# WGLab/NanoRepeat

Hardware: NVIDIA B200
Metric: GCUPS (higher is better)
Workload: dtype u16x2 (2*score + mark + 64 per half, two reads per word); s32 (score*65536 - span) for reads > 384 bases

## Files before the change

nanorepeat_b200/csrc/nr_launch_pair2.cu:

```cuda
#define NR_DEFINE_PAIR_ROUND2_KERNEL
#include "nr_launch.h"
#include <mutex>
namespace nrl {
cudaError_t launch_pair_round2(int blocks, int threads, size_t smem, cudaStream_t st, const nr::pr::Pair2* pairs,
                               const nr::pr::Deal& deal, const nr::Task* tasks, const nr::RestArgs& ra, const uint32_t* pool,
                               const nr::ScoreW& k, int* counter, int stride, int4* out, uint32_t* state) {
    static std::mutex mu;
    static bool done = false;
    {
        std::lock_guard<std::mutex> lk(mu);
        cudaError_t e = prepare(nr::pr::pair_round2_kernel, done);
        if (e != cudaSuccess) return e;
    }
    nr::pr::pair_round2_kernel<<<blocks, threads, smem, st>>>(pairs, deal, tasks, ra, pool, k, counter, stride, out, state);
    return cudaGetLastError();
}
}
```

nanorepeat_b200/csrc/nr_launch_pair3.cu:

```cuda
#define NR_DEFINE_PAIR_LADDER_KERNEL
#include "nr_launch.h"
#include <mutex>
namespace nrl {
cudaError_t launch_pair_ladder(int blocks, int threads, size_t smem, cudaStream_t st, const nr::pr::Pair3* pairs,
                               const nr::pr::Deal& deal, const nr::LadderTask* tasks, const nr::RestArgs& ra,
                               const uint32_t* qpool, const uint32_t* pool, const nr::LadderRegion* regs, const nr::ScoreW& k,
                               int* counter, int stride, uint2* prung, int4* out, int4* sel, int* redo_count, int32_t* redo,
                               const uint32_t* qstate) {
    static std::mutex mu;
    static bool done = false;
    {
        std::lock_guard<std::mutex> lk(mu);
        cudaError_t e = prepare(nr::pr::pair_ladder_kernel, done);
        if (e != cudaSuccess) return e;
    }
    nr::pr::pair_ladder_kernel<<<blocks, threads, smem, st>>>(pairs, deal, tasks, ra, qpool, pool, regs, k, counter, stride, prung,
                                                             out, sel, redo_count, redo, qstate);
    return cudaGetLastError();
}
}
```

nanorepeat_b200/csrc/nr_pair_kernels.cuh:

```cuda
#pragma once
#include "nr_kernels.cuh"

namespace nr {
namespace pr {

typedef unsigned u32;
constexpr int kBias = 64;
__host__ __device__ constexpr u32 pk2(int hi, int lo) { return ((u32)(hi & 0xffff) << 16) | (u32)(lo & 0xffff); }
__host__ __device__ constexpr u32 pk(int v) { return pk2(v, v); }
__host__ __device__ constexpr u32 sub2(int v) { return 0u - (((u32)v << 16) | (u32)v); }

constexpr int kMatch = 4, kMismatch = 8, kAmbiguous = 2, kOpen1 = 12, kExt1 = 4, kOpen2 = 50, kExt2 = 2, kRefund1 = 8, kRefund2 = 48;
constexpr u32 kFloorFwd = pk(kBias + 1);
constexpr u32 kFloorBwd = pk(kBias);
constexpr u32 kOnes = 0x00010001u;

__device__ __forceinline__ u32 pmadd(u32 a, u32 mul, u32 b) {
    u32 d;
    asm("mad.lo.u32 %0, %1, %2, %3;" : "=r"(d) : "r"(a), "r"(mul), "r"(b));
    return d;
}

template <u32 FLOOR>
__device__ __forceinline__ void cell(u32 hd, u32 s, u32 one, u32& h, u32& e1, u32& e2, u32& f1, u32& f2) {
    const u32 d = __viaddmax_u16x2(hd, s, FLOOR);
    const u32 t = __vimax3_u16x2(d, e1, e2);
    h = __vimax3_u16x2(t, f1, f2);
    e1 = __viaddmax_u16x2(h, pk(-kOpen1), pmadd(e1, one, sub2(kExt1)));
    e2 = __viaddmax_u16x2(h, pk(-kOpen2), pmadd(e2, one, sub2(kExt2)));
    f1 = __viaddmax_u16x2(h, pk(-kOpen1), pmadd(f1, one, sub2(kExt1)));
    f2 = __viaddmax_u16x2(h, pk(-kOpen2), pmadd(f2, one, sub2(kExt2)));
}

struct Pair2 {
    int32_t a, b;
    int32_t mark_col;
    int32_t state_off;
};

struct Pair3 {
    int32_t a, b;
    int32_t rung_off;
    int32_t state_off;
    int32_t R;
    int32_t pad[3];
};

__host__ __device__ constexpr int state_words(int R) { return 3 * R + 1; }

template <int R>
__device__ __forceinline__ void build_profile(uint4* prof, const uint32_t* __restrict__ qa, int q_a,
                                              const uint32_t* __restrict__ qb, int q_b, int row0, int lane, bool reverse) {
    constexpr int CH = StripeCfg<R>::CH;
    u32* p = reinterpret_cast<u32*>(prof);
    const uint32_t amb_a = q_a > 0 ? read_ambiguity_plane(qa, q_a) : 0u, amb_b = q_b > 0 ? read_ambiguity_plane(qb, q_b) : 0u;
#pragma unroll
    for (int r = 0; r < 4 * CH; ++r) {
        const int i = row0 + r;
        int ca = 4, cb = 4;
        if (r < R && i < q_a) {
            const int qi = reverse ? q_a - 1 - i : i;
            ca = (qa[qi >> 4] >> (30 - 2 * (qi & 15))) & 3;
            if (amb_a && read_base_ambiguous(qa, amb_a, qi)) ca = 5;
        }
        if (r < R && i < q_b) {
            const int qi = reverse ? q_b - 1 - i : i;
            cb = (qb[qi >> 4] >> (30 - 2 * (qi & 15))) & 3;
            if (amb_b && read_base_ambiguous(qb, amb_b, qi)) cb = 5;
        }
#pragma unroll
        for (int c = 0; c < 4; ++c)
            p[((c * CH + (r >> 2)) * 32 + lane) * 4 + (r & 3)] =
                pk2(ca == 5 ? -kAmbiguous : ca == c ? kMatch : -kMismatch, cb == 5 ? -kAmbiguous : cb == c ? kMatch : -kMismatch);
    }
}

constexpr int kP2 = 0, kPB = 1, kPF = 2;

template <int R, int MODE, bool MULTI = false>
struct Sweep {
    static constexpr u32 FLOOR = MODE == kPB ? kFloorBwd : kFloorFwd;
    static constexpr bool kMarks = MODE != kPB;
    bool top, bot;
    const ulonglong2* bnd_in;
    ulonglong2* bnd_out;
    int tag_in, tag_out;
    int* spin;
    int4 bcur;
    ulonglong2 bnxt;
    const ulonglong2* tok_in;
    ulonglong2* tok_out;
    const u32* bstage;
    int b_stride, brow0;
    const int* bdone;
    int bdone_need;
    bool late_pending;
    u32* bsm_w;
    const uint4* prof;
    const uint32_t* twords;
    int t_len, lane;
    int mark_col;
    int q_a, q_b;
    const u32* bsm;
    uint2* rung_out;
    int jnext, m, kcnt, zone_start;
    int col0;
    const u32* resume;
    u32* save;
    int save_col;
    u32 H[R], E1[R], E2[R];
    u32 hup_prev, h_out, f1_out, f2_out;
    u32 best;
    u32 bestc, raw_hi, raw_lo;
    int st_hi, st_lo;
    u32 nz, bz;
    uint32_t twl, w0, w1;
    int wi, wmax, wsh;
    const char* prof_lane;
    u32 tokP, tokJ;

    __device__ __forceinline__ uint32_t tword(int i) const { return __ldg(&twords[min(max(i, 0), wmax)]); }

    __device__ __forceinline__ void init() {
        if (MODE == kPF && resume) {
#pragma unroll
            for (int r = 0; r < R; ++r) {
                H[r] = __ldcg(&resume[r * 32 + lane]);
                E1[r] = __ldcg(&resume[(R + r) * 32 + lane]);
                E2[r] = __ldcg(&resume[(2 * R + r) * 32 + lane]);
            }
            hup_prev = lane ? __ldcg(&resume[(R - 1) * 32 + lane - 1]) : FLOOR;
            best = __ldcg(&resume[3 * R * 32 + lane]);
        } else {
#pragma unroll
            for (int r = 0; r < R; ++r) { H[r] = FLOOR; E1[r] = FLOOR + sub2(kOpen1); E2[r] = FLOOR + sub2(kOpen2); }
            hup_prev = FLOOR;
            best = 0;
        }
        h_out = FLOOR; f1_out = FLOOR; f2_out = FLOOR;
        bestc = FLOOR | kOnes; raw_hi = 0; raw_lo = 0; st_hi = 0; st_lo = 0;
        nz = lane != 0; bz = lane != 0 ? 0u : FLOOR;
        wmax = (t_len + 15) >> 4;
        wi = (col0 - lane) >> 4;
        wsh = 2 * ((col0 - lane) & 15);
        w0 = tword(wi); w1 = tword(wi + 1);
        twl = 0;
        prof_lane = reinterpret_cast<const char*>(prof + lane);
        tokP = 0; tokJ = 0;
        if (MULTI) {
            bcur = make_int4(0, 0, 0, 0); bnxt = make_ulonglong2(0ull, 0ull);
            if (top) bnxt = load_bnd(&bnd_in[lane < t_len ? lane : t_len - 1]);
            late_pending = MODE == kPF;
        }
    }

    __device__ __forceinline__ void refill() {
        twl = __funnelshift_l(w1, w0, wsh);
        w0 = w1;
        ++wi;
        w1 = tword(wi + 1);
    }

    __device__ __forceinline__ unsigned next_base(unsigned four) {
        unsigned lo, hi;
        asm("{\n\t.reg .u64 p;\n\tmul.wide.u32 p, %2, %3;\n\tmov.b64 {%0, %1}, p;\n\t}" : "=r"(lo), "=r"(hi) : "r"(twl), "r"(four));
        twl = lo;
        return hi;
    }

    template <bool JUNC, bool KEEP_E = false>
    __device__ __forceinline__ u32 cells(const uint4* pp, u32 hd, u32 cm, u32& f1, u32& f2, u32 one, u32& jhi, bool keep = false) {
        constexpr int CH = StripeCfg<R>::CH;
        u32 jprev = 0;
#pragma unroll
        for (int c = 0; c < CH; ++c) {
            const uint4 sv = pp[c * 32];
            const u32 s4[4] = {sv.x, sv.y, sv.z, sv.w};
#pragma unroll
            for (int u = 0; u < 4; ++u) {
                const int r = 4 * c + u;
                if (r < R) {
                    const u32 hleft = H[r];
                    const u32 e1pre = E1[r], e2pre = E2[r];
                    u32 h;
                    cell<FLOOR>(hd, s4[u], one, h, E1[r], E2[r], f1, f2);
                    if (KEEP_E) { E1[r] = keep ? e1pre : E1[r]; E2[r] = keep ? e2pre : E2[r]; }
                    if (JUNC) {
                        const u32 bx = bsm[(0 * R + r) * 32 + lane], by = bsm[(1 * R + r) * 32 + lane], bz = bsm[(2 * R + r) * 32 + lane];
                        const u32 t = __vimax3_u16x2(pmadd(h, one, bx), pmadd(e1pre, one, by), pmadd(e2pre, one, bz));
                        if (r & 1) jhi = __vimax3_u16x2(jhi, jprev, t);
                        else if (r == R - 1) jhi = __vmaxu2(jhi, t);
                        jprev = t;
                    }
                    hd = hleft;
                    H[r] = h;
                    if (r & 1) cm = __vimax3_u16x2(cm, h, H[r - 1]);
                    else if (r == R - 1) cm = __vmaxu2(cm, h);
                }
            }
        }
        return cm;
    }

    __device__ __forceinline__ void mark_started_inside() {
#pragma unroll
        for (int r = 0; r < R; ++r) {
            H[r] = __viaddmax_u16x2(H[r], pk(-1), FLOOR);
            E1[r] = __viaddmax_u16x2(E1[r], pk(-1), __vminu2(E1[r], FLOOR));
            E2[r] = __viaddmax_u16x2(E2[r], pk(-1), __vminu2(E2[r], FLOOR));
        }
        hup_prev = __viaddmax_u16x2(hup_prev, pk(-1), FLOOR);
    }

    __device__ __forceinline__ void late_load() {
        wait_cols(bdone, bdone_need, lane, spin);
#pragma unroll
        for (int r = 0; r < R; ++r) {
            const int idx0 = brow0 + lane * R + r;
            const int ia = q_a - 2 - idx0, ib = q_b - 2 - idx0;
#pragma unroll
            for (int c = 0; c < 3; ++c) {
                const u32 da = c == 0 ? (idx0 < q_a ? (u32)kBias : 0u) : 0u, db = c == 0 ? (idx0 < q_b ? (u32)kBias : 0u) : 0u;
                const u32 a = ia >= 0 ? __ldcg(&bstage[c * b_stride + ia]) >> 16 : da;
                const u32 b = ib >= 0 ? __ldcg(&bstage[c * b_stride + ib]) & 0xffffu : db;
                bsm_w[(c * R + r) * 32 + lane] = (a << 16) | b;
            }
        }
        __syncwarp();
        late_pending = false;
    }

    __device__ __forceinline__ void store_stage(u32* stage, int stride, int row0) {
#pragma unroll
        for (int r = 0; r < R; ++r) {
            const int i = row0 + lane * R + r;
            __stcg(&stage[0 * stride + i], H[r]);
            __stcg(&stage[1 * stride + i], E1[r] + pk(kRefund1));
            __stcg(&stage[2 * stride + i], E2[r] + pk(kRefund2));
        }
    }

    __device__ __forceinline__ void store_junction_vectors(u32* stage, u32* bvec_fwd) {
        __syncwarp();
#pragma unroll
        for (int r = 0; r < R; ++r) {
            stage[(0 * R + r) * 32 + lane] = H[r];
            stage[(1 * R + r) * 32 + lane] = E1[r] + pk(kRefund1);
            stage[(2 * R + r) * 32 + lane] = E2[r] + pk(kRefund2);
        }
        __syncwarp();
#pragma unroll
        for (int r = 0; r < R; ++r) {
            const int idx0 = lane * R + r;
            const int ia = q_a - 2 - idx0, ib = q_b - 2 - idx0;
#pragma unroll
            for (int c = 0; c < 3; ++c) {
                const u32 da = c == 0 ? (idx0 < q_a ? (u32)kBias : 0u) : 0u, db = c == 0 ? (idx0 < q_b ? (u32)kBias : 0u) : 0u;
                const u32 a = ia >= 0 ? stage[(c * R + ia % R) * 32 + ia / R] >> 16 : da;
                const u32 b = ib >= 0 ? stage[(c * R + ib % R) * 32 + ib / R] & 0xffffu : db;
                bvec_fwd[(c * R + r) * 32 + lane] = (a << 16) | b;
            }
        }
    }

    template <bool FAST, bool TRACK, bool SPECIAL = false>
    __device__ __forceinline__ void step(int st, u32 one, unsigned four) {
        const bool zone = MODE == kPF && (FAST ? SPECIAL : st >= zone_start);
        constexpr int CH = StripeCfg<R>::CH;
        u32 hup = __shfl_up_sync(kFull, h_out, 1);
        u32 f1 = __shfl_up_sync(kFull, f1_out, 1);
        u32 f2 = __shfl_up_sync(kFull, f2_out, 1);
        u32 tP = 0, tJ = 0;
        if (zone) {
            tP = __shfl_up_sync(kFull, tokP, 1);
            tJ = __shfl_up_sync(kFull, tokJ, 1);
        }
        if (MULTI && top) {
            if ((st & 31) == 0) {
                ulonglong2 raw = bnxt;
                const int cj = st + lane;
                for (int tries = 0; !__all_sync(kFull, bnd_valid(raw, tag_in) || cj >= t_len); ++tries) {
                    if (tries > kSpinLimit) { *spin = 1; break; }
                    if (tries > 3) __nanosleep(32);
                    raw = load_bnd(&bnd_in[cj < t_len ? cj : t_len - 1]);
                }
                bcur = unpack_bnd(raw);
                const int nj = st + 32 + lane;
                bnxt = load_bnd(&bnd_in[nj < t_len ? nj : t_len - 1]);
            }
            const u32 bh = __shfl_sync(kFull, (u32)bcur.x, st & 31);
            const u32 bf1 = __shfl_sync(kFull, (u32)bcur.y, st & 31);
            const u32 bf2 = __shfl_sync(kFull, (u32)bcur.z, st & 31);
            if (lane == 0) { hup = bh; f1 = bf1; f2 = bf2; }
        } else {
            hup = pmadd(hup, nz, bz);
            f1 = pmadd(f1, nz, bz);
            f2 = pmadd(f2, nz, bz);
        }
        const unsigned tb = next_base(four);
        const int rel = st - lane;
        const int jj = rel + col0;
        const bool anyj = zone && __any_sync(kFull, jj + 1 == jnext && jj < t_len);
        if (FAST || (rel >= 0 && jj < t_len)) {
            const uint4* pp = reinterpret_cast<const uint4*>(prof_lane + tb * (unsigned)(CH * 512));
            const u32 hd = hup_prev;
            hup_prev = hup;
            constexpr bool kChecks = !FAST || SPECIAL;
            const bool last_col = !FAST && MODE == kPB && jj == t_len - 1;
            u32 cm, jhi = 0;
            const u32 cm0 = (MODE == kP2 && TRACK) ? 0u : best;
            if (zone && anyj) cm = cells<true>(pp, hd, cm0, f1, f2, one, jhi);
            else if (MODE == kPB && !FAST) cm = cells<false, true>(pp, hd, cm0, f1, f2, one, jhi, last_col);
            else cm = cells<false>(pp, hd, cm0, f1, f2, one, jhi);
            h_out = H[R - 1]; f1_out = f1; f2_out = f2;
            if (MODE == kP2 && TRACK) {
                const u32 nb = __vmaxu2(bestc, cm | kOnes);
                const u32 x = nb ^ bestc;
                bestc = nb;
                if (x > 0xffffu) { st_hi = st; raw_hi = cm; }
                if (x & 0xffffu) { st_lo = st; raw_lo = cm; }
                if (kChecks && save && jj == save_col) {
#pragma unroll
                    for (int r = 0; r < R; ++r) {
                        __stcg(&save[r * 32 + lane], H[r]);
                        __stcg(&save[(R + r) * 32 + lane], E1[r]);
                        __stcg(&save[(2 * R + r) * 32 + lane], E2[r]);
                    }
                    __stcg(&save[3 * R * 32 + lane], bestc);
                }
            } else {
                best = cm;
            }
            if (zone && jj + 1 == jnext) {
                if (lane == 0) {
                    tP = 0; tJ = 0;
                    if (MULTI && top) {
                        ulonglong2 t = load_tok(&tok_in[kcnt]);
                        for (int tries = 0; (int)(t.x >> 32) != tag_in || (int)(t.y >> 32) != tag_in; ++tries) {
                            if (tries > kSpinLimit) { *spin = 1; break; }
                            if (tries > 3) __nanosleep(32);
                            t = load_tok(&tok_in[kcnt]);
                        }
                        tP = (u32)t.x; tJ = (u32)t.y;
                    }
                }
                const u32 jv = jj == mark_col ? jhi - kOnes : jhi;
                tokP = __vmaxu2(tP, best);
                tokJ = __vmaxu2(tJ, jv);
                if (lane == 31) {
                    if (MULTI && bot) __stcg(&tok_out[kcnt], make_ulonglong2(tokP | ((u64)(unsigned)tag_out << 32), tokJ | ((u64)(unsigned)tag_out << 32)));
                    else rung_out[kcnt] = make_uint2(tokP, tokJ);
                }
                jnext += m;
                ++kcnt;
            }
            if (kMarks && kChecks && jj == mark_col) mark_started_inside();
            if (MULTI && bot && lane == 31) store_bnd(&bnd_out[jj], (int)h_out, (int)f1_out, (int)f2_out, tag_out);
        }
    }

    __device__ __forceinline__ void slow_until(int& st, int end, u32 one, unsigned four) {
#pragma unroll 1
        for (; st < end; ++st) {
            if (MULTI && MODE == kPF && late_pending && st >= zone_start) late_load();
            if ((st & 15) == 0) refill();
            step<false, true>(st, one, four);
        }
    }

#ifndef NR_PAIR3_UNROLL
#define NR_PAIR3_UNROLL 2
#endif
#ifndef NR_PAIR2_UNROLL
#define NR_PAIR2_UNROLL 4
#endif
#ifndef NR_PAIR2_MULTI_UNROLL
#define NR_PAIR2_MULTI_UNROLL 4
#endif
    static constexpr int kUnroll = MODE == kP2 ? (MULTI ? NR_PAIR2_MULTI_UNROLL : NR_PAIR2_UNROLL) : (MULTI ? 1 : NR_PAIR3_UNROLL);
    template <bool TRACK, bool SPECIAL = false>
    __device__ __forceinline__ void fast_until(int& st, int end, u32 one, unsigned four) {
        for (; st + 16 <= end; st += 16) {
            refill();
#pragma unroll 1
            for (int b = 0; b < 16; b += kUnroll) {
#pragma unroll
                for (int u = 0; u < kUnroll; ++u) step<true, TRACK, SPECIAL>(st + b + u, one, four);
            }
        }
    }

    __device__ __forceinline__ void run(u32 one, unsigned four, int zone_start_) {
        init();
        zone_start = zone_start_;
        const int n = t_len - col0;
        const int nsteps = n + 31;
        const int inside_end = ((n - 1) >> 4) << 4;
        const int mc = mark_col - col0;
        int st = 0;
        slow_until(st, min(32, nsteps), one, four);
        if (MODE == kPB) {
            fast_until<true>(st, inside_end, one, four);
        } else if (MODE == kP2) {
            if (mc >= 0) {
                const int zs = max(mc - 2, 0);
                const int before = st;
                fast_until<false>(st, min(inside_end, (zs >> 4) << 4), one, four);
                if (st != before) {
                    const u32 nb = __vmaxu2(bestc, best | kOnes);
                    const u32 x = nb ^ bestc;
                    bestc = nb;
                    if (x > 0xffffu) { st_hi = lane; raw_hi = 0; }
                    if (x & 0xffffu) { st_lo = lane; raw_lo = 0; }
                }
                slow_until(st, min(nsteps, ((mc + 32 + 15) >> 4) << 4), one, four);
            }
            fast_until<true>(st, inside_end, one, four);
        } else {
            const int first = min(zone_start, mc >= 0 ? mc : zone_start);
            fast_until<true>(st, min(inside_end, (first >> 4) << 4), one, four);
            if (MULTI && late_pending && st + 16 <= inside_end) late_load();
            fast_until<true, true>(st, inside_end, one, four);
        }
        slow_until(st, nsteps, one, four);
    }
};

constexpr int kMaxRPair3 = 16;
constexpr int kMaxRPair2 = kMaxRPair3;
constexpr int kPairEntry = 1 << 30;

__host__ __device__ __forceinline__ int pair_rows(int q_len) {
    int R = (q_len + 31) / 32;
    return R < kMinR ? kMinR : R;
}

struct Deal {
    int n_rest, n_pairs;
    int static_rest;
    int nb_long;
    int static_pairs;
};
__host__ __device__ inline Deal make_deal(int n_rest, int n_pairs, int wpb, int grid) {
    Deal d;
    d.n_rest = n_rest; d.n_pairs = n_pairs;
    d.static_rest = n_rest < wpb * grid ? n_rest : wpb * grid;
    d.nb_long = (d.static_rest + wpb - 1) / wpb;
    const int room = wpb * (grid - d.nb_long);
    d.static_pairs = n_pairs < room ? n_pairs : room;
    return d;
}
__device__ __forceinline__ int next_item(const Deal& dl, bool& first, int* counter) {
    if (dl.nb_long < 0) {
        const int n = dl.n_rest + dl.n_pairs;
        if (first) {
            first = false;
            const int i = (threadIdx.x >> 5) * (int)gridDim.x + (int)blockIdx.x;
            return i < n ? i : -1;
        }
        int i = 0;
        if ((threadIdx.x & 31) == 0) i = atomicAdd(counter, 1);
        i = __shfl_sync(kFull, i, 0) + (blockDim.x >> 5) * (int)gridDim.x;
        return i < n ? i : -1;
    }
    if (first) {
        first = false;
        const int wpb = blockDim.x >> 5, warp = threadIdx.x >> 5, blk = (int)blockIdx.x;
        if (blk < dl.nb_long) {
            const int e = blk * wpb + warp;
            if (e < dl.static_rest) return e;
        } else {
            const int p = warp * ((int)gridDim.x - dl.nb_long) + (blk - dl.nb_long);
            if (p < dl.static_pairs) return dl.n_rest + p;
        }
    }
    int d = 0;
    if ((threadIdx.x & 31) == 0) d = atomicAdd(counter, 1);
    d = __shfl_sync(kFull, d, 0);
    const int rest_left = dl.n_rest - dl.static_rest;
    if (d < rest_left) return dl.static_rest + d;
    const int p = dl.static_pairs + d - rest_left;
    return p < dl.n_pairs ? dl.n_rest + p : -1;
}

template <int R>
__device__ __forceinline__ void pair2_task(const Pair2& pt, const Task* __restrict__ tasks, const uint32_t* __restrict__ pool,
                                           uint4* prof, int lane, u32 one, unsigned four, int4* out, u32* state) {
    const Task ta = tasks[pt.a];
    Task tb = ta;
    int q_b = 0;
    if (pt.b >= 0) { tb = tasks[pt.b]; q_b = tb.q_len; }
    __syncwarp();
    build_profile<R>(prof, pool + ta.q_word, ta.q_len, pool + tb.q_word, q_b, lane * R, lane, false);
    __syncwarp();
    Sweep<R, kP2> sw;
    sw.prof = prof; sw.twords = pool + ta.t_word; sw.t_len = ta.t_len; sw.lane = lane;
    sw.mark_col = pt.mark_col;
    sw.col0 = 0; sw.resume = nullptr;
    sw.save_col = pt.mark_col - 2;
    sw.save = (state && pt.state_off >= 0 && sw.save_col >= 0) ? state + (size_t)pt.state_off * 32 : nullptr;
    sw.run(one, four, 0);
#pragma unroll
    for (int half = 0; half < 2; ++half) {
        const u32 cls = half ? (sw.bestc & 0xffffu) : (sw.bestc >> 16);
        const u32 raw = half ? (sw.raw_lo & 0xffffu) : (sw.raw_hi >> 16);
        const int st = half ? sw.st_lo : sw.st_hi;
        const int score = (int)(cls - (kBias + 1)) >> 1;
        const int col = st - lane;
        unsigned key = 0;
        if (score > 0) key = ((unsigned)score << 17) | ((0xffffu - (unsigned)col) << 1) | (raw & 1u);
        key = __reduce_max_sync(kFull, key);
        const int tid = half ? pt.b : pt.a;
        if (lane == 0 && tid >= 0) {
            int4 rec = make_int4(0, 0, 0, 0);
            if (key) {
                const int c = 0xffff - (int)((key >> 1) & 0xffffu);
                const bool inside = c <= pt.mark_col || !(key & 1u);
                rec = make_int4((int)(key >> 17), inside ? 0 : pt.mark_col + 1, c + 1, 0);
            }
            out[tid] = rec;
        }
    }
}

template <int R>
__device__ __noinline__ void pair2_stripe(const Pair2& pt, int s, const Task* __restrict__ tasks, const uint32_t* __restrict__ pool,
                                          const RestArgs& ra, uint4* prof, int lane, u32 one, unsigned four, int4* out) {
    const CoopInfo ci = ra.coop[pt.state_off];
    const int S = ci.n_stripes;
    int* F = ra.flags + ci.flag_off;
    ulonglong2* bnd_a = reinterpret_cast<ulonglong2*>(ra.scratch + ci.data_off);
    ulonglong2* bnd_b = bnd_a + ci.bnd_stride;
    const Task ta = tasks[pt.a];
    Task tb = ta;
    int q_b = 0;
    if (pt.b >= 0) { tb = tasks[pt.b]; q_b = tb.q_len; }
    __syncwarp();
    build_profile<R>(prof, pool + ta.q_word, ta.q_len, pool + tb.q_word, q_b, s * 32 * R + lane * R, lane, false);
    __syncwarp();
    Sweep<R, kP2, true> sw;
    sw.prof = prof; sw.twords = pool + ta.t_word; sw.t_len = ta.t_len; sw.lane = lane;
    sw.mark_col = pt.mark_col;
    sw.col0 = 0; sw.resume = nullptr; sw.save = nullptr; sw.save_col = -1;
    sw.top = s > 0; sw.bot = s + 1 < S;
    sw.bnd_in = (s & 1) ? bnd_a : bnd_b; sw.bnd_out = (s & 1) ? bnd_b : bnd_a;
    sw.tag_in = stripe_tag(ra.epoch, s - 1); sw.tag_out = stripe_tag(ra.epoch, s); sw.spin = ra.spin;
    sw.run(one, four, 0);
    unsigned keys[2];
#pragma unroll
    for (int half = 0; half < 2; ++half) {
        const u32 cls = half ? (sw.bestc & 0xffffu) : (sw.bestc >> 16);
        const u32 raw = half ? (sw.raw_lo & 0xffffu) : (sw.raw_hi >> 16);
        const int st = half ? sw.st_lo : sw.st_hi;
        const int score = (int)(cls - (kBias + 1)) >> 1;
        unsigned key = 0;
        if (score > 0) key = ((unsigned)score << 17) | ((0xffffu - (unsigned)(st - lane)) << 1) | (raw & 1u);
        keys[half] = __reduce_max_sync(kFull, key);
    }
    if (lane == 0) {
        unsigned* K = reinterpret_cast<unsigned*>(F + 2 * S + 2);
        atomicMax(&K[0], keys[0]);
        atomicMax(&K[1], keys[1]);
        __threadfence();
        if (atomicAdd(F + 2 * S, 1) == S - 1) {
            __threadfence();
#pragma unroll
            for (int half = 0; half < 2; ++half) {
                const int tid = half ? pt.b : pt.a;
                if (tid < 0) continue;
                const unsigned key = atomicMax(&K[half], 0u);
                int4 rec = make_int4(0, 0, 0, 0);
                if (key) {
                    const int c = 0xffff - (int)((key >> 1) & 0xffffu);
                    const bool inside = c <= pt.mark_col || !(key & 1u);
                    rec = make_int4((int)(key >> 17), inside ? 0 : pt.mark_col + 1, c + 1, 0);
                }
                out[tid] = rec;
            }
        }
    }
}

template <int R>
__device__ __forceinline__ void pair2_stripe_dispatch(int r, const Pair2& pt, int s, const Task* __restrict__ tasks,
                                                      const uint32_t* __restrict__ pool, const RestArgs& ra, uint4* prof, int lane,
                                                      u32 one, unsigned four, int4* out) {
    if constexpr (is_coop_height(R))
        if (r == R) { pair2_stripe<R>(pt, s, tasks, pool, ra, prof, lane, one, four, out); return; }
    if constexpr (R < kMaxRLadder) pair2_stripe_dispatch<R + 1>(r, pt, s, tasks, pool, ra, prof, lane, one, four, out);
}

template <int R>
__device__ __forceinline__ void pair2_dispatch(int r, const Pair2& pt, const Task* __restrict__ tasks,
                                               const uint32_t* __restrict__ pool, uint4* prof, int lane, u32 one,
                                               unsigned four, int4* out, u32* state) {
    if (r == R) { pair2_task<R>(pt, tasks, pool, prof, lane, one, four, out, state); return; }
    if constexpr (R < kMaxRPair2) pair2_dispatch<R + 1>(r, pt, tasks, pool, prof, lane, one, four, out, state);
}

#ifdef NR_DEFINE_PAIR_ROUND2_KERNEL
__global__ void __launch_bounds__(32 * kWarpsPerBlock, 1)
pair_round2_kernel(const Pair2* __restrict__ pairs, Deal dl, const Task* __restrict__ tasks, RestArgs ra,
                   const uint32_t* __restrict__ pool, ScoreW scw, int* counter, int smem_stride, int4* out, u32* state) {
    extern __shared__ uint4 psmem[];
    const ScoreView<true> sc(scw);
    const int lane = threadIdx.x & 31, warp = threadIdx.x >> 5;
    uint4* prof = psmem + warp * smem_stride;
    bool first = true;
    for (;;) {
        const int i = next_item(dl, first, counter);
        if (i < 0) break;
        if (i < ra.n_order) {
            const int e = ra.order[i];
            if (e & kPairEntry) {
                const Pair2 mp = pairs[(e & ~kPairEntry) >> kCodeBits];
                pair2_stripe_dispatch<kMinR>(ra.coop[mp.state_off].rows, mp, (e & ((1 << kCodeBits) - 1)) - 1, tasks, pool, ra, prof, lane,
                                             (u32)sc.one, sc.four, out);
            } else {
                exact_entry(e, tasks, pool, sc, ra, reinterpret_cast<int4*>(prof), lane, out);
            }
            continue;
        }
        const Pair2 pt = pairs[i - ra.n_order];
        int q = tasks[pt.a].q_len;
        if (pt.b >= 0) q = max(q, tasks[pt.b].q_len);
        pair2_dispatch<kMinR>(pair_rows(q), pt, tasks, pool, prof, lane, (u32)sc.one, sc.four, out, state);
    }
}
#endif

__device__ __forceinline__ void rung_of(u32 P, u32 J, u32 rc, int& score, bool& in_right, bool& unmarked) {
    const u32 np = max(J, rc);
    const int s_p = (int)(P - kBias) >> 1;
    const int s_np = (int)(np - 2 * kBias) >> 1;
    in_right = s_np > s_p;
    score = max(s_p, s_np);
    unmarked = np & 1u;
}

__device__ __forceinline__ void pair3_select(const Pair3& pt, const LadderTask& ta, const LadderTask& tb, int kmin, u32 rcand,
                                             const uint2* rungs, int lane, int min_score, int4* sel, int* redo_count, int32_t* redo,
                                             int redo_shift) {
#pragma unroll
    for (int half = 0; half < 2; ++half) {
        const int tid = half ? pt.b : pt.a;
        if (tid < 0) continue;
        const LadderTask& tk = half ? tb : ta;
        const u32 rc = half ? (rcand & 0xffffu) : (rcand >> 16);
        int top = 0;
        for (int k = tk.kmin + lane; k <= tk.kmax; k += 32) {
            const uint2 t = rungs[k - kmin];
            int s; bool ir, um;
            rung_of(half ? (t.x & 0xffffu) : (t.x >> 16), half ? (t.y & 0xffffu) : (t.y >> 16), rc, s, ir, um);
            if (s >= min_score) top = max(top, s);
        }
        top = __reduce_max_sync(kFull, top);
        int n = 0, sum = 0, unsure = 0;
        if (top > 0) {
            for (int k = tk.kmin + lane; k <= tk.kmax; k += 32) {
                const uint2 t = rungs[k - kmin];
                int s; bool ir, um;
                rung_of(half ? (t.x & 0xffffu) : (t.x >> 16), half ? (t.y & 0xffffu) : (t.y >> 16), rc, s, ir, um);
                if (s == top && ir) {
                    if (um) unsure = 1;
                    else { ++n; sum += k; }
                }
            }
        }
        n = __reduce_add_sync(kFull, n);
        sum = __reduce_add_sync(kFull, sum);
        unsure = __any_sync(kFull, unsure);
        if (lane == 0) {
            sel[tk.read] = make_int4(top, n, sum, 0);
            if (unsure) redo[atomicAdd(redo_count, 1)] = tid << redo_shift;
        }
    }
}

template <int R>
__device__ __forceinline__ void pair3_task(const Pair3& pt, const LadderTask* __restrict__ tasks,
                                           const uint32_t* __restrict__ qpool, const uint32_t* __restrict__ pool,
                                           const LadderRegion* __restrict__ regs, uint4* prof, int lane, u32 one,
                                           unsigned four, int min_score, uint2* prung, int4* sel, int* redo_count,
                                           int32_t* redo, const u32* __restrict__ qstate) {
    const bool ha = pt.a >= 0, hb = pt.b >= 0;
    const LadderTask tv = tasks[ha ? pt.a : pt.b];
    LadderTask ta = tv, tb = tv;
    int q_a = 0, q_b = 0;
    if (ha) { ta = tasks[pt.a]; q_a = ta.q_len; }
    if (hb) { tb = tasks[pt.b]; q_b = tb.q_len; }
    const LadderRegion reg = regs[tv.region];
    const int kmin = (ha && hb) ? min(ta.kmin, tb.kmin) : tv.kmin;
    const int kmax = (ha && hb) ? max(ta.kmax, tb.kmax) : tv.kmax;
    u32* bsm = reinterpret_cast<u32*>(prof + StripeCfg<R>::PROF_INT4);
    uint2* rungs = prung + pt.rung_off;
    __syncwarp();
    build_profile<R>(prof, qpool + ta.q_word, q_a, qpool + tb.q_word, q_b, lane * R, lane, true);
    __syncwarp();
    u32 rcand;
    {
        Sweep<R, kPB> sw;
        sw.prof = prof; sw.twords = pool + reg.rev_word; sw.t_len = reg.n_right; sw.lane = lane;
        sw.mark_col = -1; sw.q_a = q_a; sw.q_b = q_b;
        sw.col0 = 0; sw.resume = nullptr; sw.save = nullptr; sw.save_col = -1;
        sw.run(one, four, 0);
        const u32 ra = __reduce_max_sync(kFull, sw.best >> 16), rb = __reduce_max_sync(kFull, sw.best & 0xffffu);
        rcand = pk2((int)ra + kBias + 1, (int)rb + kBias + 1);
        sw.store_junction_vectors(reinterpret_cast<u32*>(prof), bsm);
    }
    __syncwarp();
    build_profile<R>(prof, qpool + ta.q_word, q_a, qpool + tb.q_word, q_b, lane * R, lane, false);
    __syncwarp();
    {
        Sweep<R, kPF> sw;
        sw.prof = prof; sw.twords = pool + reg.fwd_word; sw.t_len = reg.n_left + reg.m * kmax; sw.lane = lane;
        sw.mark_col = reg.n_left - 1; sw.bsm = bsm; sw.rung_out = rungs;
        sw.m = reg.m; sw.jnext = reg.n_left + reg.m * kmin; sw.kcnt = 0;
        sw.save = nullptr; sw.save_col = -1;
        const bool resumes = qstate && pt.state_off >= 0;
        sw.col0 = resumes ? reg.n_left - 1 : 0;
        sw.resume = resumes ? qstate + (size_t)pt.state_off * 32 : nullptr;
        sw.run(one, four, sw.jnext - 1 - sw.col0);
    }
    __syncwarp();
    pair3_select(pt, ta, tb, kmin, rcand, rungs, lane, min_score, sel, redo_count, redo, kCodeBits);
}

template <int R>
__device__ __noinline__ void pair3_bwd_stripe(const Pair3& pt, int s, const LadderTask* __restrict__ tasks,
                                              const uint32_t* __restrict__ qpool, const uint32_t* __restrict__ pool,
                                              const LadderRegion* __restrict__ regs, const RestArgs& ra, uint4* prof, int lane,
                                              u32 one, unsigned four) {
    const CoopInfo ci = ra.coop[pt.pad[0]];
    const int S = ci.n_stripes;
    int* F = ra.flags + ci.flag_off;
    ulonglong2* bnd_a = reinterpret_cast<ulonglong2*>(ra.scratch + ci.data_off);
    ulonglong2* bnd_b = bnd_a + ci.bnd_stride;
    u32* stage = reinterpret_cast<u32*>(ra.scratch + ci.data_off + 4 * ci.bnd_stride);
    const LadderTask ta = tasks[pt.a], tb = tasks[pt.b];
    const LadderRegion reg = regs[ta.region];
    __syncwarp();
    build_profile<R>(prof, qpool + ta.q_word, ta.q_len, qpool + tb.q_word, tb.q_len, s * 32 * R + lane * R, lane, true);
    __syncwarp();
    Sweep<R, kPB, true> sw;
    sw.prof = prof; sw.twords = pool + reg.rev_word; sw.t_len = reg.n_right; sw.lane = lane;
    sw.mark_col = -1; sw.q_a = ta.q_len; sw.q_b = tb.q_len;
    sw.col0 = 0; sw.resume = nullptr; sw.save = nullptr; sw.save_col = -1;
    sw.top = s > 0; sw.bot = s + 1 < S;
    sw.bnd_in = (s & 1) ? bnd_a : bnd_b; sw.bnd_out = (s & 1) ? bnd_b : bnd_a;
    sw.tag_in = stripe_tag(ra.epoch, s - 1); sw.tag_out = stripe_tag(ra.epoch, s); sw.spin = ra.spin;
    sw.run(one, four, 0);
    sw.store_stage(stage, ci.b_stride, s * 32 * R);
    const u32 ba = __reduce_max_sync(kFull, sw.best >> 16), bb = __reduce_max_sync(kFull, sw.best & 0xffffu);
    __syncwarp();
    if (lane == 0) {
        unsigned* K = reinterpret_cast<unsigned*>(F + 2 * S + 2);
        atomicMax(&K[0], ba);
        atomicMax(&K[1], bb);
        __threadfence();
        atomicAdd(F + 2 * S, 1);
    }
}

template <int R>
__device__ __noinline__ void pair3_fwd_stripe(const Pair3& pt, int s, const LadderTask* __restrict__ tasks,
                                              const uint32_t* __restrict__ qpool, const uint32_t* __restrict__ pool,
                                              const LadderRegion* __restrict__ regs, const RestArgs& ra, uint4* prof, int lane,
                                              u32 one, unsigned four, int min_score, uint2* prung, int4* sel, int* redo_count,
                                              int32_t* redo) {
    const CoopInfo ci = ra.coop[pt.pad[0]];
    const int S = ci.n_stripes;
    int* F = ra.flags + ci.flag_off;
    ulonglong2* bnd_a = reinterpret_cast<ulonglong2*>(ra.scratch + ci.data_off + 2 * ci.bnd_stride);
    ulonglong2* bnd_b = bnd_a + ci.bnd_stride;
    const u32* stage = reinterpret_cast<const u32*>(ra.scratch + ci.data_off + 4 * ci.bnd_stride);
    ulonglong2* tok_a = reinterpret_cast<ulonglong2*>(ra.scratch + ci.data_off + 4 * ci.bnd_stride + (3 * ci.b_stride + 3) / 4);
    ulonglong2* tok_b = tok_a + ci.tok_stride;
    const LadderTask ta = tasks[pt.a], tb = tasks[pt.b];
    const LadderRegion reg = regs[ta.region];
    const int kmin = min(ta.kmin, tb.kmin), kmax = max(ta.kmax, tb.kmax);
    u32* bsm = reinterpret_cast<u32*>(prof + StripeCfg<R>::PROF_INT4);
    uint2* rungs = prung + pt.rung_off;
    __syncwarp();
    build_profile<R>(prof, qpool + ta.q_word, ta.q_len, qpool + tb.q_word, tb.q_len, s * 32 * R + lane * R, lane, false);
    __syncwarp();
    Sweep<R, kPF, true> sw;
    sw.prof = prof; sw.twords = pool + reg.fwd_word; sw.t_len = reg.n_left + reg.m * kmax; sw.lane = lane;
    sw.mark_col = reg.n_left - 1; sw.bsm = bsm; sw.bsm_w = bsm; sw.rung_out = rungs;
    sw.m = reg.m; sw.jnext = reg.n_left + reg.m * kmin; sw.kcnt = 0;
    sw.q_a = ta.q_len; sw.q_b = tb.q_len;
    sw.save = nullptr; sw.save_col = -1; sw.col0 = 0; sw.resume = nullptr;
    sw.top = s > 0; sw.bot = s + 1 < S;
    sw.bnd_in = (s & 1) ? bnd_a : bnd_b; sw.bnd_out = (s & 1) ? bnd_b : bnd_a;
    sw.tok_in = (s & 1) ? tok_a : tok_b; sw.tok_out = (s & 1) ? tok_b : tok_a;
    sw.tag_in = stripe_tag(ra.epoch, s - 1); sw.tag_out = stripe_tag(ra.epoch, s); sw.spin = ra.spin;
    sw.bstage = stage; sw.b_stride = ci.b_stride; sw.brow0 = s * 32 * R;
    sw.bdone = F + 2 * S; sw.bdone_need = S;
    sw.run(one, four, sw.jnext - 1);
    if (s == S - 1) {
        __syncwarp();
        if (sw.late_pending) wait_cols(sw.bdone, sw.bdone_need, lane, ra.spin);
        const unsigned* K = reinterpret_cast<const unsigned*>(F + 2 * S + 2);
        const u32 rcand = pk2((int)__ldcg(&K[0]) + kBias + 1, (int)__ldcg(&K[1]) + kBias + 1);
        pair3_select(pt, ta, tb, kmin, rcand, rungs, lane, min_score, sel, ra.redo_long_count, ra.redo_long, 0);
    }
}

template <int R>
__device__ __forceinline__ void pair3_stripe_dispatch(int r, const Pair3& pt, int code, const LadderTask* __restrict__ tasks,
                                                      const uint32_t* __restrict__ qpool, const uint32_t* __restrict__ pool,
                                                      const LadderRegion* __restrict__ regs, const RestArgs& ra, uint4* prof,
                                                      int lane, u32 one, unsigned four, int min_score, uint2* prung, int4* sel,
                                                      int* redo_count, int32_t* redo) {
    if constexpr (is_coop_height(R))
        if (r == R) {
            if (code < kCodeFwd) pair3_bwd_stripe<R>(pt, code - 1, tasks, qpool, pool, regs, ra, prof, lane, one, four);
            else pair3_fwd_stripe<R>(pt, code - kCodeFwd, tasks, qpool, pool, regs, ra, prof, lane, one, four, min_score, prung, sel,
                                     redo_count, redo);
            return;
        }
    if constexpr (R < kMaxRLadder)
        pair3_stripe_dispatch<R + 1>(r, pt, code, tasks, qpool, pool, regs, ra, prof, lane, one, four, min_score, prung, sel, redo_count, redo);
}

template <int R>
__device__ __forceinline__ void pair3_dispatch(int r, const Pair3& pt, const LadderTask* __restrict__ tasks,
                                               const uint32_t* __restrict__ qpool, const uint32_t* __restrict__ pool,
                                               const LadderRegion* __restrict__ regs, uint4* prof, int lane, u32 one,
                                               unsigned four, int min_score, uint2* prung, int4* sel, int* redo_count,
                                               int32_t* redo, const u32* __restrict__ qstate) {
    if (r == R) { pair3_task<R>(pt, tasks, qpool, pool, regs, prof, lane, one, four, min_score, prung, sel, redo_count, redo, qstate); return; }
    if constexpr (R < kMaxRPair3)
        pair3_dispatch<R + 1>(r, pt, tasks, qpool, pool, regs, prof, lane, one, four, min_score, prung, sel, redo_count, redo, qstate);
}

#ifdef NR_DEFINE_PAIR_LADDER_KERNEL
__global__ void __launch_bounds__(32 * kWarpsPerBlock, 1)
pair_ladder_kernel(const Pair3* __restrict__ pairs, Deal dl, const LadderTask* __restrict__ tasks, RestArgs ra,
                   const uint32_t* __restrict__ qpool, const uint32_t* __restrict__ pool,
                   const LadderRegion* __restrict__ regs, ScoreW scw, int* counter,
                   int smem_stride, uint2* prung, int4* out, int4* sel, int* redo_count, int32_t* redo,
                   const u32* __restrict__ qstate) {
    extern __shared__ uint4 psmem[];
    const ScoreView<true> sc(scw);
    const int lane = threadIdx.x & 31, warp = threadIdx.x >> 5;
    uint4* prof = psmem + warp * smem_stride;
    bool first = true;
    for (;;) {
        const int i = next_item(dl, first, counter);
        if (i < 0) break;
        if (i < ra.n_order) {
            const int e = ra.order[i];
            if (e & kPairEntry) {
                const Pair3 mp = pairs[(e & ~kPairEntry) >> kCodeBits];
                pair3_stripe_dispatch<kMinR>(mp.R, mp, e & ((1 << kCodeBits) - 1), tasks, qpool, pool, regs, ra, prof, lane, (u32)sc.one,
                                             sc.four, sc.min_score, prung, sel, redo_count, redo);
            } else {
                ladder_entry<true, kMaxRLadder>(e, tasks, qpool, pool, regs, sc, ra, reinterpret_cast<int4*>(prof), lane, out, sel);
            }
            continue;
        }
        const Pair3 pt = pairs[i - ra.n_order];
        int rows = pt.R;
        if (rows <= 0) {
            int q = pt.a >= 0 ? tasks[pt.a].q_len : 0;
            if (pt.b >= 0) q = max(q, tasks[pt.b].q_len);
            rows = pair_rows(q);
        }
        pair3_dispatch<kMinR>(rows, pt, tasks, qpool, pool, regs, prof, lane, (u32)sc.one, sc.four, sc.min_score, prung, sel, redo_count, redo, qstate);
    }
}
#endif

}
}
```

Before: 66100.

## Specialise ramp-in/out sweep steps and cache junction vectors in registers

Adds dedicated ramp-in and ramp-out step variants that drop the per-step boundary, save and mark checks when they provably cannot fire, replacing the generic slow path at the start and end of each sweep. For the forward ladder sweep with small row counts, the junction vectors are loaded once into registers instead of being re-read from shared memory on every junction cell. Per-phase clock instrumentation is added behind a compile flag, so it is off by default. The register cache raises register pressure, and the ramp variants add code size and extra guard conditions.

```diff
diff --git a/nanorepeat_b200/csrc/nr_launch_pair2.cu b/nanorepeat_b200/csrc/nr_launch_pair2.cu
--- a/nanorepeat_b200/csrc/nr_launch_pair2.cu
+++ b/nanorepeat_b200/csrc/nr_launch_pair2.cu
@@ -16,3 +16,14 @@
     return cudaGetLastError();
 }
 }
+
+#ifdef NR_PHASE_CLOCKS
+extern "C" int nr_phase_clocks_pair_round2(unsigned long long* out, int reset) {
+    cudaError_t e = cudaMemcpyFromSymbol(out, nr::pr::g_phase_clk, sizeof(nr::pr::g_phase_clk));
+    if (e == cudaSuccess && reset) {
+        const unsigned long long zero[nr::pr::kPhases] = {};
+        e = cudaMemcpyToSymbol(nr::pr::g_phase_clk, zero, sizeof(zero));
+    }
+    return (int)e;
+}
+#endif
diff --git a/nanorepeat_b200/csrc/nr_launch_pair3.cu b/nanorepeat_b200/csrc/nr_launch_pair3.cu
--- a/nanorepeat_b200/csrc/nr_launch_pair3.cu
+++ b/nanorepeat_b200/csrc/nr_launch_pair3.cu
@@ -19,3 +19,14 @@
     return cudaGetLastError();
 }
 }
+
+#ifdef NR_PHASE_CLOCKS
+extern "C" int nr_phase_clocks_pair_ladder(unsigned long long* out, int reset) {
+    cudaError_t e = cudaMemcpyFromSymbol(out, nr::pr::g_phase_clk, sizeof(nr::pr::g_phase_clk));
+    if (e == cudaSuccess && reset) {
+        const unsigned long long zero[nr::pr::kPhases] = {};
+        e = cudaMemcpyToSymbol(nr::pr::g_phase_clk, zero, sizeof(zero));
+    }
+    return (int)e;
+}
+#endif
diff --git a/nanorepeat_b200/csrc/nr_pair_kernels.cuh b/nanorepeat_b200/csrc/nr_pair_kernels.cuh
--- a/nanorepeat_b200/csrc/nr_pair_kernels.cuh
+++ b/nanorepeat_b200/csrc/nr_pair_kernels.cuh
@@ -76,6 +76,34 @@
 }
 
 constexpr int kP2 = 0, kPB = 1, kPF = 2;
+
+enum Phase { kPhProfile, kPhRampIn, kPhSteady, kPhZone, kPhRampOut, kPhJvec, kPhSelect, kPhIdle, kPhMid, kPhOther, kPhases };
+#ifdef NR_PHASE_CLOCKS
+static __device__ unsigned long long g_phase_clk[kPhases];
+__device__ __forceinline__ long long& phase_last() {
+    __shared__ long long last[kWarpsPerBlock];
+    return last[threadIdx.x >> 5];
+}
+__device__ __forceinline__ void phase_mark(int ph) {
+    if ((threadIdx.x & 31) == 0) {
+        const long long t = clock64();
+        if (ph >= 0) atomicAdd(&g_phase_clk[ph], (unsigned long long)(t - phase_last()));
+        phase_last() = t;
+    }
+}
+__device__ __forceinline__ void phase_idle() {
+    __shared__ long long end_max;
+    phase_mark(kPhOther);
+    if (threadIdx.x == 0) end_max = 0;
+    __syncthreads();
+    if ((threadIdx.x & 31) == 0) atomicMax(&end_max, phase_last());
+    __syncthreads();
+    if ((threadIdx.x & 31) == 0) atomicAdd(&g_phase_clk[kPhIdle], (unsigned long long)(end_max - phase_last()));
+}
+#else
+__device__ __forceinline__ void phase_mark(int) {}
+__device__ __forceinline__ void phase_idle() {}
+#endif
 
 template <int R, int MODE, bool MULTI = false>
 struct Sweep {
@@ -95,6 +123,9 @@
     const int* bdone;
     int bdone_need;
     bool late_pending;
+    static constexpr bool kJReg = MODE == kPF && !MULTI && R <= 12;
+    u32 JB[kJReg ? 3 * R : 1];
+    bool ramp_marks;
     u32* bsm_w;
     const uint4* prof;
     const uint32_t* twords;
@@ -168,7 +199,7 @@
         return hi;
     }
 
-    template <bool JUNC, bool KEEP_E = false>
+    template <bool JUNC, bool KEEP_E = false, bool JREG = false>
     __device__ __forceinline__ u32 cells(const uint4* pp, u32 hd, u32 cm, u32& f1, u32& f2, u32 one, u32& jhi, bool keep = false) {
         constexpr int CH = StripeCfg<R>::CH;
         u32 jprev = 0;
@@ -186,7 +217,12 @@
                     cell<FLOOR>(hd, s4[u], one, h, E1[r], E2[r], f1, f2);
                     if (KEEP_E) { E1[r] = keep ? e1pre : E1[r]; E2[r] = keep ? e2pre : E2[r]; }
                     if (JUNC) {
-                        const u32 bx = bsm[(0 * R + r) * 32 + lane], by = bsm[(1 * R + r) * 32 + lane], bz = bsm[(2 * R + r) * 32 + lane];
+                        u32 bx, by, bz;
+                        if constexpr (JREG && kJReg) {
+                            bx = JB[r]; by = JB[R + r]; bz = JB[2 * R + r];
+                        } else {
+                            bx = bsm[(0 * R + r) * 32 + lane]; by = bsm[(1 * R + r) * 32 + lane]; bz = bsm[(2 * R + r) * 32 + lane];
+                        }
                         const u32 t = __vimax3_u16x2(pmadd(h, one, bx), pmadd(e1pre, one, by), pmadd(e2pre, one, bz));
                         if (r & 1) jhi = __vimax3_u16x2(jhi, jprev, t);
                         else if (r == R - 1) jhi = __vmaxu2(jhi, t);
@@ -212,6 +248,13 @@
         hup_prev = __viaddmax_u16x2(hup_prev, pk(-1), FLOOR);
     }
 
+    __device__ __forceinline__ void load_jvec() {
+        if constexpr (kJReg) {
+#pragma unroll
+            for (int i = 0; i < 3 * R; ++i) JB[i] = bsm[i * 32 + lane];
+        }
+    }
+
     __device__ __forceinline__ void late_load() {
         wait_cols(bdone, bdone_need, lane, spin);
 #pragma unroll
@@ -263,9 +306,10 @@
         }
     }
 
-    template <bool FAST, bool TRACK, bool SPECIAL = false>
+    static constexpr int kRampIn = 1, kRampOut = 2;
+    template <bool FAST, bool TRACK, bool SPECIAL = false, int RAMP = 0>
     __device__ __forceinline__ void step(int st, u32 one, unsigned four) {
-        const bool zone = MODE == kPF && (FAST ? SPECIAL : st >= zone_start);
+        const bool zone = MODE == kPF && (FAST ? SPECIAL : RAMP == kRampIn ? false : RAMP == kRampOut ? true : st >= zone_start);
         constexpr int CH = StripeCfg<R>::CH;
         u32 hup = __shfl_up_sync(kFull, h_out, 1);
         u32 f1 = __shfl_up_sync(kFull, f1_out, 1);
@@ -300,17 +344,18 @@
         const unsigned tb = next_base(four);
         const int rel = st - lane;
         const int jj = rel + col0;
-        const bool anyj = zone && __any_sync(kFull, jj + 1 == jnext && jj < t_len);
-        if (FAST || (rel >= 0 && jj < t_len)) {
+        const bool anyj = zone && (RAMP == kRampOut || __any_sync(kFull, jj + 1 == jnext && jj < t_len));
+        if (FAST || (RAMP == kRampIn ? rel >= 0 : RAMP == kRampOut ? jj < t_len : (rel >= 0 && jj < t_len))) {
             const uint4* pp = reinterpret_cast<const uint4*>(prof_lane + tb * (unsigned)(CH * 512));
             const u32 hd = hup_prev;
             hup_prev = hup;
-            constexpr bool kChecks = !FAST || SPECIAL;
-            const bool last_col = !FAST && MODE == kPB && jj == t_len - 1;
+            constexpr bool kChecks = (!FAST || SPECIAL) && RAMP != kRampOut;
+            constexpr bool kSaveChecks = kChecks && RAMP == 0;
+            const bool last_col = !FAST && RAMP != kRampIn && MODE == kPB && jj == t_len - 1;
             u32 cm, jhi = 0;
             const u32 cm0 = (MODE == kP2 && TRACK) ? 0u : best;
-            if (zone && anyj) cm = cells<true>(pp, hd, cm0, f1, f2, one, jhi);
-            else if (MODE == kPB && !FAST) cm = cells<false, true>(pp, hd, cm0, f1, f2, one, jhi, last_col);
+            if (zone && anyj) cm = cells<true, false, (SPECIAL || RAMP == kRampOut)>(pp, hd, cm0, f1, f2, one, jhi);
+            else if (MODE == kPB && !FAST && RAMP != kRampIn) cm = cells<false, true>(pp, hd, cm0, f1, f2, one, jhi, last_col);
             else cm = cells<false>(pp, hd, cm0, f1, f2, one, jhi);
             h_out = H[R - 1]; f1_out = f1; f2_out = f2;
             if (MODE == kP2 && TRACK) {
@@ -319,7 +364,7 @@
                 bestc = nb;
                 if (x > 0xffffu) { st_hi = st; raw_hi = cm; }
                 if (x & 0xffffu) { st_lo = st; raw_lo = cm; }
-                if (kChecks && save && jj == save_col) {
+                if (kSaveChecks && save && jj == save_col) {
 #pragma unroll
                     for (int r = 0; r < R; ++r) {
                         __stcg(&save[r * 32 + lane], H[r]);
@@ -354,7 +399,7 @@
                 jnext += m;
                 ++kcnt;
             }
-            if (kMarks && kChecks && jj == mark_col) mark_started_inside();
+            if (kMarks && kChecks && (RAMP != kRampIn || ramp_marks) && jj == mark_col) mark_started_inside();
             if (MULTI && bot && lane == 31) store_bnd(&bnd_out[jj], (int)h_out, (int)f1_out, (int)f2_out, tag_out);
         }
     }
@@ -390,6 +435,16 @@
         }
     }
 
+    template <int RAMP>
+    __device__ __forceinline__ void ramp(int& st, int end, u32 one, unsigned four) {
+        for (; st < end; st += 16) {
+            refill();
+#pragma unroll 1
+            for (int b = 0; b < 16 && st + b < end; ++b) step<false, true, false, RAMP>(st + b, one, four);
+        }
+        st = end;
+    }
+
     __device__ __forceinline__ void run(u32 one, unsigned four, int zone_start_) {
         init();
         zone_start = zone_start_;
@@ -398,9 +453,14 @@
         const int inside_end = ((n - 1) >> 4) << 4;
         const int mc = mark_col - col0;
         int st = 0;
-        slow_until(st, min(32, nsteps), one, four);
+        const bool save_in = MODE == kP2 && save && save_col >= col0 && save_col < col0 + 32;
+        ramp_marks = kMarks && mc >= 0 && mc < 32;
+        if (!MULTI && n > 32 && !save_in && (MODE != kPF || zone_start >= 32)) ramp<kRampIn>(st, 32, one, four);
+        else slow_until(st, min(32, nsteps), one, four);
+        phase_mark(kPhRampIn);
         if (MODE == kPB) {
             fast_until<true>(st, inside_end, one, four);
+            phase_mark(kPhSteady);
         } else if (MODE == kP2) {
             if (mc >= 0) {
                 const int zs = max(mc - 2, 0);
@@ -413,16 +473,28 @@
                     if (x > 0xffffu) { st_hi = lane; raw_hi = 0; }
                     if (x & 0xffffu) { st_lo = lane; raw_lo = 0; }
                 }
+                phase_mark(kPhSteady);
                 slow_until(st, min(nsteps, ((mc + 32 + 15) >> 4) << 4), one, four);
+                phase_mark(kPhMid);
             }
             fast_until<true>(st, inside_end, one, four);
+            phase_mark(kPhSteady);
         } else {
             const int first = min(zone_start, mc >= 0 ? mc : zone_start);
             fast_until<true>(st, min(inside_end, (first >> 4) << 4), one, four);
+            phase_mark(kPhSteady);
             if (MULTI && late_pending && st + 16 <= inside_end) late_load();
+            load_jvec();
             fast_until<true, true>(st, inside_end, one, four);
-        }
-        slow_until(st, nsteps, one, four);
+            phase_mark(kPhZone);
+        }
+        const int behind = col0 + st - 31;
+        const bool marks_out = kMarks && mark_col >= behind && mark_col < t_len;
+        const bool save_out = MODE == kP2 && save && save_col >= behind && save_col < t_len;
+        if (!MULTI && st >= 32 && (st & 15) == 0 && !marks_out && !save_out && (MODE != kPF || zone_start <= st))
+            ramp<kRampOut>(st, nsteps, one, four);
+        else slow_until(st, nsteps, one, four);
+        phase_mark(kPhRampOut);
     }
 };
 
@@ -490,9 +562,11 @@
     Task tb = ta;
     int q_b = 0;
     if (pt.b >= 0) { tb = tasks[pt.b]; q_b = tb.q_len; }
+    phase_mark(kPhOther);
     __syncwarp();
     build_profile<R>(prof, pool + ta.q_word, ta.q_len, pool + tb.q_word, q_b, lane * R, lane, false);
     __syncwarp();
+    phase_mark(kPhProfile);
     Sweep<R, kP2> sw;
     sw.prof = prof; sw.twords = pool + ta.t_word; sw.t_len = ta.t_len; sw.lane = lane;
     sw.mark_col = pt.mark_col;
@@ -521,6 +595,7 @@
             out[tid] = rec;
         }
     }
+    phase_mark(kPhSelect);
 }
 
 template <int R>
@@ -607,6 +682,7 @@
     const int lane = threadIdx.x & 31, warp = threadIdx.x >> 5;
     uint4* prof = psmem + warp * smem_stride;
     bool first = true;
+    phase_mark(-1);
     for (;;) {
         const int i = next_item(dl, first, counter);
         if (i < 0) break;
@@ -619,6 +695,7 @@
             } else {
                 exact_entry(e, tasks, pool, sc, ra, reinterpret_cast<int4*>(prof), lane, out);
             }
+            phase_mark(kPhOther);
             continue;
         }
         const Pair2 pt = pairs[i - ra.n_order];
@@ -626,6 +703,7 @@
         if (pt.b >= 0) q = max(q, tasks[pt.b].q_len);
         pair2_dispatch<kMinR>(pair_rows(q), pt, tasks, pool, prof, lane, (u32)sc.one, sc.four, out, state);
     }
+    phase_idle();
 }
 #endif
 
@@ -694,9 +772,11 @@
     const int kmax = (ha && hb) ? max(ta.kmax, tb.kmax) : tv.kmax;
     u32* bsm = reinterpret_cast<u32*>(prof + StripeCfg<R>::PROF_INT4);
     uint2* rungs = prung + pt.rung_off;
+    phase_mark(kPhOther);
     __syncwarp();
     build_profile<R>(prof, qpool + ta.q_word, q_a, qpool + tb.q_word, q_b, lane * R, lane, true);
     __syncwarp();
+    phase_mark(kPhProfile);
     u32 rcand;
     {
         Sweep<R, kPB> sw;
@@ -708,9 +788,11 @@
         rcand = pk2((int)ra + kBias + 1, (int)rb + kBias + 1);
         sw.store_junction_vectors(reinterpret_cast<u32*>(prof), bsm);
     }
+    phase_mark(kPhJvec);
     __syncwarp();
     build_profile<R>(prof, qpool + ta.q_word, q_a, qpool + tb.q_word, q_b, lane * R, lane, false);
     __syncwarp();
+    phase_mark(kPhProfile);
     {
         Sweep<R, kPF> sw;
         sw.prof = prof; sw.twords = pool + reg.fwd_word; sw.t_len = reg.n_left + reg.m * kmax; sw.lane = lane;
@@ -724,6 +806,7 @@
     }
     __syncwarp();
     pair3_select(pt, ta, tb, kmin, rcand, rungs, lane, min_score, sel, redo_count, redo, kCodeBits);
+    phase_mark(kPhSelect);
 }
 
 template <int R>
@@ -846,6 +929,7 @@
     const int lane = threadIdx.x & 31, warp = threadIdx.x >> 5;
     uint4* prof = psmem + warp * smem_stride;
     bool first = true;
+    phase_mark(-1);
     for (;;) {
         const int i = next_item(dl, first, counter);
         if (i < 0) break;
@@ -858,6 +942,7 @@
             } else {
                 ladder_entry<true, kMaxRLadder>(e, tasks, qpool, pool, regs, sc, ra, reinterpret_cast<int4*>(prof), lane, out, sel);
             }
+            phase_mark(kPhOther);
             continue;
         }
         const Pair3 pt = pairs[i - ra.n_order];
@@ -869,6 +954,7 @@
         }
         pair3_dispatch<kMinR>(rows, pt, tasks, qpool, pool, regs, prof, lane, (u32)sc.one, sc.four, sc.min_score, prung, sel, redo_count, redo, qstate);
     }
+    phase_idle();
 }
 #endif
 
```

Measured after the change: 65490, median of 6. About the same (-0.9%).
